# ingonyama-zk/icicle-snark

Measured on AMD Instinct MI355X. Metric: groth16_prove_constraints_per_s, higher is better.
Workload: dtype u256 mod p (MSM: 9x29-bit limbs in u32, Montgomery R=2^261, lazy reduction; NTT: 9x29-bit limbs, lazy; QAP/vec ops: 8xu32 limbs, Montgomery R=2^256)

## Files before the change

icicle-snark_amd/binding.py:

```python
from __future__ import annotations

import ctypes as C
import os

import numpy as np

_HERE = os.path.dirname(os.path.abspath(__file__))
LIB_PATH = os.path.join(_HERE, "lib", "libicicle_snark_hip.so")
os.environ.setdefault("GPU_MAX_HW_QUEUES", "12")

SUCCESS = 0
ERRORS = ["SUCCESS", "INVALID_DEVICE", "OUT_OF_MEMORY", "INVALID_POINTER", "ALLOCATION_FAILED", "DEALLOCATION_FAILED",
          "COPY_FAILED", "SYNCHRONIZATION_FAILED", "STREAM_CREATION_FAILED", "STREAM_DESTRUCTION_FAILED",
          "API_NOT_IMPLEMENTED", "INVALID_ARGUMENT", "BACKEND_LOAD_FAILED", "LICENSE_CHECK_ERROR", "UNKNOWN_ERROR"]


class IcicleError(RuntimeError):
    def __init__(self, code, what=""):
        self.code = code
        name = ERRORS[code] if 0 <= code < len(ERRORS) else str(code)
        super().__init__(f"eIcicleError::{name} {what}".strip())


class Device(C.Structure):
# ... 45 lines not shown
icicle_copy_to_host_async icicle_copy_to_device icicle_copy_to_device_async icicle_create_stream icicle_destroy_stream
icicle_stream_synchronize icicle_device_synchronize icicle_get_device_properties
create_config_extension destroy_config_extension config_extension_set_int config_extension_set_bool
config_extension_get_int config_extension_get_bool clone_config_extension
bn254_generate_scalars bn254_add bn254_sub bn254_mul bn254_inv bn254_pow bn254_from_u32
bn254_eq bn254_ecadd bn254_ecsub bn254_mul_scalar bn254_to_affine bn254_from_affine bn254_generator bn254_is_on_curve
bn254_base_field_from_u32 bn254_g2_eq bn254_g2_ecadd bn254_g2_ecsub bn254_g2_mul_scalar bn254_g2_to_affine
bn254_g2_from_affine bn254_g2_generator bn254_g2_is_on_curve bn254_g2_base_field_from_u32
bn254_vector_add bn254_vector_sub bn254_vector_mul bn254_scalar_convert_montgomery
bn254_affine_convert_montgomery bn254_g2_affine_convert_montgomery
bn254_ntt bn254_ntt_init_domain bn254_ntt_release_domain bn254_get_root_of_unity bn254_get_root_of_unity_from_domain
bn254_msm bn254_g2_msm bn254_pairing
bn254_vector_div bn254_vector_accumulate bn254_vector_sum bn254_vector_product bn254_scalar_add_vec bn254_scalar_sub_vec
bn254_scalar_mul_vec bn254_projective_convert_montgomery bn254_g2_projective_convert_montgomery
bn254_msm_precompute_bases bn254_g2_msm_precompute_bases
bn254_pairing_target_field_add bn254_pairing_target_field_sub bn254_pairing_target_field_mul bn254_pairing_target_field_inv
bn254_pairing_target_field_pow bn254_pairing_target_field_from_u32 bn254_pairing_target_field_generate_scalars
icicle_snark_last_error icicle_snark_g1_generator_mul icicle_snark_g2_generator_mul icicle_snark_last_msm_timings
icicle_snark_msm_profile icicle_snark_microbench icicle_snark_pmc_probes icicle_snark_access_probes
icicle_snark_pairing_batch icicle_snark_pairing_product icicle_snark_msm_segmented
""".split()

_lib = None


def lib():
    global _lib
    if _lib is None:
        if not os.path.exists(LIB_PATH):
            raise ImportError(f"{LIB_PATH} is missing: run `make` (hipcc --offload-arch=gfx950); "
                              "this package has no CPU fallback")
        _lib = C.CDLL(LIB_PATH)
        _lib.icicle_snark_last_error.restype = C.c_char_p
        _lib.groth16_last_error.restype = _lib.groth16_verify_last_error.restype = C.c_char_p
        _lib.groth16_cache_manager_new.restype = C.c_void_p
        _lib.groth16_zkey_export_vk.restype = C.c_int64
        _lib.groth16_verify_combined_coefficients.restype = _lib.groth16_vkset_free.restype = None
        for n in ("bn254_eq", "bn254_g2_eq", "bn254_is_on_curve", "bn254_g2_is_on_curve"):
            getattr(_lib, n).restype = C.c_bool
    return _lib


def check(rc, what=""):
    if rc != SUCCESS:
        msg = lib().icicle_snark_last_error()
        raise IcicleError(rc, f"{what}: {msg.decode() if msg else ''}")


def set_device(dev_type: str = "HIP", dev_id: int = 0):
    if dev_type != "CPU":
        check(lib().icicle_load_backend_from_env_or_default(), "load_backend")
    d = Device(dev_type.encode(), dev_id)
    check(lib().icicle_set_device(C.byref(d)), f"set_device({dev_type},{dev_id})")


def ptr_of(a):
    if a is None:
        return None
    if isinstance(a, np.ndarray):
        assert a.flags["C_CONTIGUOUS"]
        return a.ctypes.data_as(C.c_void_p)
    if isinstance(a, DeviceVec):
        return C.c_void_p(a.ptr)
    if isinstance(a, int):
        return C.c_void_p(a)
    raise TypeError(type(a))


def _on_dev(a):
    return isinstance(a, (DeviceVec, int))


class IcicleStream:

    def __init__(self, handle=None):
        if handle is None:
            h = C.c_void_p()
            check(lib().icicle_create_stream(C.byref(h)), "create_stream")
            self.handle, self._own = h.value, True
        else:
            self.handle, self._own = handle, False

    def synchronize(self):
        check(lib().icicle_stream_synchronize(C.c_void_p(self.handle)), "stream_synchronize")

    def destroy(self):
        if self._own and self.handle is not None:
            check(lib().icicle_destroy_stream(C.c_void_p(self.handle)), "destroy_stream")
            self.handle = None


class DeviceVec:

    def __init__(self, nbytes: int, stream: IcicleStream | None = None, _ptr=None, _parent=None):
        self.nbytes = nbytes
        self._parent = _parent
        if _ptr is not None:
            self.ptr = _ptr
            return
        p = C.c_void_p()
        if stream is None:
            check(lib().icicle_malloc(C.byref(p), C.c_size_t(max(nbytes, 1))), "malloc")
        else:
            check(lib().icicle_malloc_async(C.byref(p), C.c_size_t(max(nbytes, 1)), C.c_void_p(stream.handle)), "malloc_async")
        self.ptr = p.value

# ... 1402 lines not shown
```

icicle-snark_amd/csrc/common.h:

```cpp
#pragma once
#include <atomic>
#include <chrono>
#include <condition_variable>
#include <hip/hip_runtime.h>
#include <mutex>
#include <stdint.h>
#include <stdio.h>
#include <stdlib.h>
#include <string>
#include <vector>

#include "../../include/icicle_snark_hip.h"

namespace isnark {

void set_last_error(const char* fmt, ...);

inline const char* env_str(const char* name) { return getenv(name); }
inline bool env_set(const char* name) { return getenv(name) != nullptr; }
inline int env_int(const char* name, int dflt)
{
  const char* v = getenv(name);
  return v ? atoi(v) : dflt;
}
inline long long env_i64(const char* name, long long dflt)
{
  const char* v = getenv(name);
  return v ? atoll(v) : dflt;
}

inline double ms_since(std::chrono::steady_clock::time_point t0)
{
  return std::chrono::duration<double, std::milli>(std::chrono::steady_clock::now() - t0).count();
}

#define ISNARK_API extern "C" __attribute__((visibility("default")))

#define HIP_TRY(call, code)                                                                                   \
  do {                                                                                                        \
    hipError_t e__ = (call);                                                                                  \
    if (e__ != hipSuccess) {                                                                                  \
      ::isnark::set_last_error("%s failed: %s (%s:%d)", #call, hipGetErrorString(e__), __FILE__, __LINE__);   \
      return (code);                                                                                          \
    }                                                                                                         \
  } while (0)

#define ICICLE_TRY(call)                                                                                      \
  do {                                                                                                        \
    eIcicleError e__ = (call);                                                                                \
    if (e__ != ICICLE_SUCCESS) return e__;                                                                    \
  } while (0)

eIcicleError require_device();
bool is_tracked_device_ptr(const void* p);
void prewarm_device(int dev, int n_streams);
bool probe_stream_pipes(hipStream_t* st, int n, int* cls);
void stream_pipes_measure(hipStream_t* st, int n);
bool stream_pipe_classes(hipStream_t* st, int n, int* cls, bool allow_measure = true);
void stream_pipes_forget(hipStream_t st);
void prewarm_modules(int dev);
void module_warm_csr(hipStream_t s);
void module_warm_qap(hipStream_t s);
void module_warm_sort(hipStream_t s);
void module_warm_g1(hipStream_t s);
void module_warm_g2(hipStream_t s);
void module_warm_g2acc(hipStream_t s);
void module_warm_ntt(hipStream_t s);
void module_warm_vec(hipStream_t s);
int default_device_or_none();
void release_cached_device_memory();

struct CopyJob {
  void* dst;
  const void* src;
  size_t n;
};
constexpr int STAGED_LANES = 8;
constexpr size_t STAGED_CHUNK_BYTES = 2u << 20;
struct StagedProgress {
  size_t head_bytes = 0;
  hipEvent_t ev[STAGED_LANES] = {};
  std::atomic<int> lanes_total{-1};
  std::atomic<int> lanes_reported{0};
  std::atomic<bool> done{false};
  std::mutex m;
  std::condition_variable cv;
  void notify()
  {
    std::lock_guard<std::mutex> lk(m);
    cv.notify_all();
  }
  void wait_head()
  {
    std::unique_lock<std::mutex> lk(m);
    cv.wait(lk, [this] {
      const int tot = lanes_total.load(std::memory_order_acquire);
      return (tot >= 0 && lanes_reported.load(std::memory_order_acquire) >= tot) || done.load(std::memory_order_acquire);
    });
  }
};
hipError_t staged_copy(int device_id, const CopyJob* jobs, size_t njobs, bool to_device, const hipStream_t* lanes = nullptr, int n_lanes = 0, bool own_temp_streams = false,
                       StagedProgress* progress = nullptr);
void staged_copy_file_hint(const void* base, size_t len, int fd);
void staged_copy_file_hint_get(const void** base, size_t* len, int* fd);
bool is_pinned_host(const void* host_ptr, int device_id = -1);
constexpr size_t STAGED_MIN_BYTES = 4u << 20;

void note_device_write(const void* p, size_t bytes);

class Staged
{
// ... 139 lines not shown
```

icicle-snark_amd/csrc/microbench.hip:

```cpp
#include <map>
#include <string.h>
#include <mutex>

#include "common.h"

using namespace isnark;

namespace {
__global__ __launch_bounds__(256) void mad_rate_kernel(uint64_t* out, const uint32_t* in, int iters)
{
  const uint32_t a = in[threadIdx.x & 7], b = in[(threadIdx.x + 1) & 7];
  uint64_t c0 = a, c1 = b, c2 = a + 1, c3 = b + 1, c4 = 5, c5 = 6, c6 = 7, c7 = 8;
  for (int it = 0; it < iters; it++) {
#pragma unroll
    for (int u = 0; u < 8; u++) {
      c0 += (uint64_t)a * b; c1 += (uint64_t)a * b; c2 += (uint64_t)a * b; c3 += (uint64_t)a * b;
      c4 += (uint64_t)a * b; c5 += (uint64_t)a * b; c6 += (uint64_t)a * b; c7 += (uint64_t)a * b;
      asm volatile("" : "+v"(c0), "+v"(c1), "+v"(c2), "+v"(c3), "+v"(c4), "+v"(c5), "+v"(c6), "+v"(c7));
    }
  }
  out[blockIdx.x * blockDim.x + threadIdx.x] = c0 ^ c1 ^ c2 ^ c3 ^ c4 ^ c5 ^ c6 ^ c7;
}
__device__ __forceinline__ uint32_t probe_hash(uint32_t x)
{
// ... 107 lines not shown
  if (le != ICICLE_SUCCESS) return le;
  return se == hipSuccess ? ICICLE_SUCCESS : ICICLE_SYNCHRONIZATION_FAILED;
}

ISNARK_API eIcicleError icicle_snark_microbench(double out[2])
{
  if (!out) return ICICLE_INVALID_POINTER;
  ICICLE_TRY(require_device());
  hipEvent_t e0, e1;
  HIP_TRY(hipEventCreate(&e0), ICICLE_UNKNOWN_ERROR);
  HIP_TRY(hipEventCreate(&e1), ICICLE_UNKNOWN_ERROR);
  const size_t bytes = (size_t)1 << 30;
  void *a = nullptr, *b = nullptr;
  HIP_TRY(hipMalloc(&a, bytes), ICICLE_ALLOCATION_FAILED);
  HIP_TRY(hipMalloc(&b, bytes), ICICLE_ALLOCATION_FAILED);
  HIP_TRY(hipMemsetAsync(a, 1, bytes, nullptr), ICICLE_UNKNOWN_ERROR);
  HIP_TRY(hipMemcpyAsync(b, a, bytes, hipMemcpyDeviceToDevice, nullptr), ICICLE_COPY_FAILED);
  HIP_TRY(hipEventRecord(e0, nullptr), ICICLE_UNKNOWN_ERROR);
  for (int i = 0; i < 4; i++) HIP_TRY(hipMemcpyAsync(b, a, bytes, hipMemcpyDeviceToDevice, nullptr), ICICLE_COPY_FAILED);
  HIP_TRY(hipEventRecord(e1, nullptr), ICICLE_UNKNOWN_ERROR);
  HIP_TRY(hipEventSynchronize(e1), ICICLE_SYNCHRONIZATION_FAILED);
  float ms = 0;
  (void)hipEventElapsedTime(&ms, e0, e1);
  out[0] = 4.0 * 2.0 * (double)bytes / (ms * 1e-3) / 1e9;
  const int blocks = 4096, iters = 500;
  hipLaunchKernelGGL(mad_rate_kernel, dim3(blocks), dim3(256), 0, nullptr, (uint64_t*)b, (const uint32_t*)a, iters);
  HIP_TRY(hipEventRecord(e0, nullptr), ICICLE_UNKNOWN_ERROR);
  hipLaunchKernelGGL(mad_rate_kernel, dim3(blocks), dim3(256), 0, nullptr, (uint64_t*)b, (const uint32_t*)a, iters);
  HIP_TRY(hipEventRecord(e1, nullptr), ICICLE_UNKNOWN_ERROR);
  HIP_TRY(hipEventSynchronize(e1), ICICLE_SYNCHRONIZATION_FAILED);
  (void)hipEventElapsedTime(&ms, e0, e1);
  out[1] = (double)blocks * 256 * iters * 64.0 / (ms * 1e-3) / 1e12;
  (void)hipFree(a);
  (void)hipFree(b);
  (void)hipEventDestroy(e0);
  (void)hipEventDestroy(e1);
  return ICICLE_SUCCESS;
}

namespace {
__global__ __launch_bounds__(256) void pipe_probe_big_kernel(unsigned long long* out, int iters)
{
  unsigned long long x = threadIdx.x + blockIdx.x;
  for (int i = 0; i < iters; i++) x = x * 6364136223846793005ull + 1442695040888963407ull;
  if (x == 42) out[0] = x;
}
__global__ void pipe_probe_tiny_kernel(unsigned long long* out)
{
  if (threadIdx.x == 999) out[1] = 1;
}
}

namespace isnark {
bool probe_stream_pipes(hipStream_t* st, int n, int* cls)
{
  for (int i = 0; i < n; i++) cls[i] = -1;
  if (n < 2 || n > 16) return false;
  unsigned long long* d = nullptr;
  if (hipMalloc((void**)&d, 64) != hipSuccess) {
    (void)hipGetLastError();
    return false;
  }
  hipEvent_t ref = nullptr, big_end = nullptr, stop[16] = {};
  bool ok = hipEventCreate(&ref) == hipSuccess && hipEventCreate(&big_end) == hipSuccess;
  for (int i = 0; i < n && ok; i++) ok = hipEventCreate(&stop[i]) == hipSuccess;
  for (int i = 0; i < n && ok; i++) {
    hipLaunchKernelGGL(pipe_probe_tiny_kernel, dim3(1), dim3(64), 0, st[i], d);
    ok = hipStreamSynchronize(st[i]) == hipSuccess;
  }
  if (ok) {
    hipLaunchKernelGGL(pipe_probe_big_kernel, dim3(64), dim3(256), 0, st[0], d, 8);
    ok = hipStreamSynchronize(st[0]) == hipSuccess;
  }
  int next_class = 0;
  for (int x = 0; x < n && ok; x++) {
    if (cls[x] >= 0) continue;
    if (next_class >= 4) {
      ok = false;
      break;
    }
    if (next_class == 3) {
      for (int j = x; j < n; j++)
        if (cls[j] < 0) cls[j] = 3;
      break;
    }
    cls[x] = next_class;
    ok = hipEventRecord(ref, st[x]) == hipSuccess;
    hipLaunchKernelGGL(pipe_probe_big_kernel, dim3(40000), dim3(256), 0, st[x], d, 3000);
    ok = ok && hipEventRecord(big_end, st[x]) == hipSuccess;
    for (int j = 0; j < n && ok; j++) {
      if (j == x) continue;
      hipLaunchKernelGGL(pipe_probe_tiny_kernel, dim3(1), dim3(64), 0, st[j], d);
      ok = hipEventRecord(stop[j], st[j]) == hipSuccess;
    }
    for (int j = 0; j < n && ok; j++) ok = hipStreamSynchronize(st[j]) == hipSuccess;
    float big_ms = 0;
    ok = ok && hipEventElapsedTime(&big_ms, ref, big_end) == hipSuccess;
    for (int j = 0; j < n && ok; j++) {
      if (j == x) continue;
      float ms = 0;
      ok = hipEventElapsedTime(&ms, ref, stop[j]) == hipSuccess;
      const bool mate = ms > 0.35f && ms > 0.1f * big_ms;
      if (mate) {
        if (cls[j] >= 0 && cls[j] != next_class) ok = false;
        cls[j] = next_class;
      }
    }
    next_class++;
  }
  (void)hipGetLastError();
  if (ref) (void)hipEventDestroy(ref);
  if (big_end) (void)hipEventDestroy(big_end);
  for (int i = 0; i < n; i++)
    if (stop[i]) (void)hipEventDestroy(stop[i]);
  (void)hipFree(d);
  if (!ok)
    for (int i = 0; i < n; i++) cls[i] = -1;
  return ok;
}

namespace {
std::mutex g_pipe_mu;
std::map<hipStream_t, std::pair<int, int>> g_pipe_cls;
int g_pipe_epoch = 0;
}
void stream_pipes_measure(hipStream_t* st, int n)
{
  int cls[16], prev[16];
  if (n > 16) n = 16;
  bool have_prev = false, agreed = false;
  for (int attempt = 0; attempt < 4 && !agreed; attempt++) {
    if (!probe_stream_pipes(st, n, cls)) {
      have_prev = false;
      continue;
    }
    agreed = have_prev && memcmp(cls, prev, sizeof(int) * n) == 0;
    memcpy(prev, cls, sizeof(int) * n);
    have_prev = true;
  }
  if (!agreed) return;
  std::lock_guard<std::mutex> lk(g_pipe_mu);
  const int ep = ++g_pipe_epoch;
  for (int i = 0; i < n; i++) g_pipe_cls[st[i]] = {ep, cls[i]};
}
bool stream_pipe_classes(hipStream_t* st, int n, int* cls, bool allow_measure)
{
  for (int attempt = 0; attempt < (allow_measure ? 2 : 1); attempt++) {
    {
      std::lock_guard<std::mutex> lk(g_pipe_mu);
      int ep = -1;
      bool all = true;
      for (int i = 0; i < n && all; i++) {
        const auto it = g_pipe_cls.find(st[i]);
        if (it == g_pipe_cls.end() || (ep >= 0 && it->second.first != ep)) all = false;
        else {
          ep = it->second.first;
          cls[i] = it->second.second;
        }
      }
      if (all) return true;
    }
    if (attempt == 0) stream_pipes_measure(st, n);
  }
  for (int i = 0; i < n; i++) cls[i] = -1;
  return false;
}
void stream_pipes_forget(hipStream_t st)
{
  std::lock_guard<std::mutex> lk(g_pipe_mu);
  g_pipe_cls.erase(st);
}
}
```

icicle-snark_amd/csrc/prover/cache.cpp:

```cpp
#include <algorithm>
#include <utility>

#include "prover_internal.h"

using namespace bn254;
using namespace isnark;
using namespace isnark::prover;

namespace isnark {
namespace prover {

ZKeyCache::~ZKeyCache()
  {
    int prev = -1;
    if (hipGetDevice(&prev) != hipSuccess) prev = -1;
    struct Restore { int d; ~Restore() { if (d >= 0) (void)hipSetDevice(d); } } restore{prev};
    (void)hipSetDevice(device_id);
    tb.cancel.store(true);
    if (tb.th.joinable()) tb.th.join();
    for (void* t : tb.fresh)
      if (t) (void)hipFree(t);
    for (hipStream_t st : streams())
      if (st) (void)hipStreamSynchronize(st);
    for (void* p : {(void*)d_rowptr, (void*)d_cols, (void*)d_vals, A.d_points, B1.d_points, B2.d_points, C.d_points, H.d_points, (void*)d_witness, (void*)d_vec, (void*)d_fold, (void*)d_skeys, (void*)d_dist_y, (void*)d_dist_recv1, (void*)d_dist_send2, (void*)d_tw1, (void*)d_partials, (void*)d_wtnz})
      if (p) (void)hipFree(p);
    if (h_partials) (void)hipHostFree(h_partials);
    for (hipStream_t st : streams())
      if (st) (void)icicle_destroy_stream(st);
    for (hipEvent_t e : {ev_witness, ev_sort, ev_sort_h, ev_own_slice, ev_head_in, ev_head_done, ev_t_head_start, ev_t_head_end, ev_t_witness})
      if (e) (void)hipEventDestroy(e);
    for (auto e : ev)
      if (e) (void)hipEventDestroy(e);
    for (auto e : ev_done)
      if (e) (void)hipEventDestroy(e);
    for (auto e : ev_lfork)
      if (e) (void)hipEventDestroy(e);
    for (auto e : ev_ljoin)
      if (e) (void)hipEventDestroy(e);
    for (auto& p : prof) msm_profile_own_destroy(&p);
  }

namespace {
G1::P g1_from_mont_affine(const uint8_t* p)
{
  G1::A a;
  memcpy(&a, p, 64);
  if (G1::aff_is_zero(a)) return {Fq::zero(), Fq::one_std(), Fq::zero()};
  return {Fq::from_mont(a.x), Fq::from_mont(a.y), Fq::one_std()};
}
G2::P g2_from_mont_affine(const uint8_t* p)
{
  G2::A a;
  memcpy(&a, p, 128);
  fe2 one = {Fq::one_std(), Fq::zero()};
  if (G2::aff_is_zero(a)) return {Fq2Ops::zero(), one, Fq2Ops::zero()};
  return {Fq2Ops::from_mont(a.x), Fq2Ops::from_mont(a.y), one};
}

struct BaseArray {
  Shard ZKeyCache::*shard;
  int section;
  bool g2;
  bool h;
  size_t elem() const { return g2 ? 128 : 64; }
  Shard& of(ZKeyCache* z) const { return z->*shard; }
  const MsmGeom& geom(const MsmGeom& gw, const MsmGeom& gh) const { return h ? gh : gw; }
};
const BaseArray BASES[5] = {{&ZKeyCache::A, 5, false, false}, {&ZKeyCache::B1, 6, false, false}, {&ZKeyCache::B2, 7, true, false}, {&ZKeyCache::C, 8, false, false}, {&ZKeyCache::H, 9, false, true}};

uint64_t witness_row_bytes(const ZKeyCache* z) { return ((uint64_t)z->A.len() + z->B1.len() + z->C.len()) * 64 + (uint64_t)z->B2.len() * 128; }

eIcicleError points_to_internal(bool g2, const Shard& sh, int from_form, hipStream_t s)
{
  return g2 ? msm_g2_points_to_internal(sh.d_points, sh.len(), from_form, s) : msm_g1_points_to_internal(sh.d_points, sh.len(), from_form, s);
}
eIcicleError build_table(bool g2, const Shard& sh, int from_form, const MsmGeom& g, hipStream_t s, void** table)
{
  return g2 ? msm_g2_build_table(sh.d_points, sh.len(), from_form, g, s, table) : msm_g1_build_table(sh.d_points, sh.len(), from_form, g, s, table);
}
eIcicleError build_table_sliced(bool g2, const Shard& sh, int from_form, const MsmGeom& g, hipStream_t s, void** table, const std::atomic<bool>* cancel)
{
  return g2 ? msm_g2_build_table_sliced(sh.d_points, sh.len(), from_form, g, s, table, cancel) : msm_g1_build_table_sliced(sh.d_points, sh.len(), from_form, g, s, table, cancel);
}
}

int staged_upload(int device_id, const std::vector<UploadJob>& jobs, const hipStream_t* lanes_in, int n_lanes, StagedProgress* progress)
{
  const hipError_t e = staged_copy(device_id, jobs.data(), jobs.size(), true, lanes_in, n_lanes, lanes_in == nullptr, progress);
  if (e != hipSuccess) return fail((int)ICICLE_COPY_FAILED, "host to device upload: %s", hipGetErrorString(e));
  return 0;
}

MsmGeom witness_table_geometry(uint32_t len)
{
  MsmGeom g = msm_geometry(len, 0, 1);
  if (!g.tab) return g;
  int c = g.c;
  while (c > 17 && (((uint64_t)len * (uint64_t)(254 / c + 1)) >> (c - 1)) < 28) c--;
  if (c != g.c) {
    const MsmGeom h = msm_geometry(len, 0, c);
    if (h.tab && h.c == c) return h;
  }
  return g;
}

namespace {
void assign_stream_roles(ZKeyCache* z, bool allow_measure)
{
  static const bool off = env_int("ICICLE_SNARK_PIPE_ROLES", 1) == 0;
  if (off) return;
  std::array<hipStream_t, 6> phys = z->streams();
  int cls[6];
  if (!stream_pipe_classes(phys.data(), 6, cls, allow_measure)) return;
  auto cost = [&](const int* perm) {
    auto same = [&](int a, int b) { return cls[perm[a]] == cls[perm[b]] ? 1 : 0; };
    int c = 1000 * (same(0, 2) + same(0, 3) + same(2, 3)) + 200 * (same(2, 1) + same(2, 4) + same(2, 5) + same(3, 1) + same(3, 4) + same(3, 5)) + 100 * (1 - same(0, 4)) +
            100 * (1 - same(1, 5));
    for (int r = 0; r < 6; r++) c += perm[r] != r ? 1 : 0;
    return c;
  };
  int perm[6] = {0, 1, 2, 3, 4, 5}, best[6] = {0, 1, 2, 3, 4, 5};
  int best_cost = cost(perm);
  while (std::next_permutation(perm, perm + 6)) {
    const int c = cost(perm);
    if (c < best_cost) {
      best_cost = c;
      memcpy(best, perm, sizeof best);
    }
  }
  int r = 0;
  for (hipStream_t* role : {&z->s_qap, &z->s_g1, &z->s_g2, &z->s_g3, &z->s_g4, &z->s_g5}) *role = phys[best[r++]];
  if (env_set("ICICLE_SNARK_TRACE_COLD") || env_set("ICICLE_SNARK_VERBOSE"))
    fprintf(stderr, "[icicle-snark-hip] stream pipes %d %d %d %d %d %d -> roles (qap A B2 Hsort B1 C) take streams %d %d %d %d %d %d (cost %d)\n", cls[0], cls[1], cls[2], cls[3], cls[4], cls[5], best[0],
            best[1], best[2], best[3], best[4], best[5], best_cost);
}
}

namespace {
void table_build_thread(ZKeyCache* z)
{
  TableBuild& tb = z->tb;
  while (tb.hold.load(std::memory_order_acquire) && !tb.cancel.load()) std::this_thread::sleep_for(std::chrono::milliseconds(1));
  const int grace_ms = env_int("ICICLE_SNARK_TABLE_GRACE_MS", TABLE_BUILD_GRACE_MS);
  for (int waited = 0; !tb.witness_only && waited < grace_ms && !tb.go.load(std::memory_order_acquire) && !tb.cancel.load(); waited++) std::this_thread::sleep_for(std::chrono::milliseconds(1));
  const auto t0 = std::chrono::steady_clock::now();
  static const bool trace_tb = env_set("ICICLE_SNARK_TRACE_TABLES");
  bool ok = hipSetDevice(z->device_id) == hipSuccess;
  if (trace_tb) fprintf(stderr, "[tables] thread: device set at %.1f ms\n", ms_since(t0));
  const MsmGeom gw_dense = tb.gw;
  bool narrowed = false;
  if (ok && !tb.witness_only && tb.go.load(std::memory_order_acquire) && z->witness_entries) {
    int lg = 0;
    while (((uint64_t)1 << lg) * 32 < z->witness_entries) lg++;
    int c_t = lg + 1 < 13 ? 13 : lg + 1;
    if (c_t < tb.gw.c) {
      const MsmGeom g = msm_geometry(z->A.len(), 0, c_t);
      if (g.tab && g.c == c_t && g.W > tb.gw.W) {
        const uint64_t per_row = witness_row_bytes(z);
        const uint64_t extra = (uint64_t)(g.W - tb.gw.W) * per_row;
        size_t free_b = 0, total_b = 0;
        const bool mem_ok = hipMemGetInfo(&free_b, &total_b) == hipSuccess && (uint64_t)g.W * per_row + (uint64_t)tb.gh.W * z->H.len() * 64 + (1ull << 30) <= free_b;
        (void)hipGetLastError();
        if (mem_ok && extra <= tb.narrow_room.load(std::memory_order_acquire)) {
          tb.gw = g;
          tb.extra_bytes.store(extra, std::memory_order_release);
          narrowed = true;
        }
      } else if (g.tab && g.c == c_t)
        tb.gw = g;
    }
  }
  hipStream_t s = nullptr;
  if (ok) {
    int least = 0, greatest = 0;
    if (hipDeviceGetStreamPriorityRange(&least, &greatest) != hipSuccess) least = 0;
    if (hipStreamCreateWithPriority(&s, hipStreamNonBlocking, least) != hipSuccess) {
      (void)hipGetLastError();
      ok = false;
    }
  }
  if (trace_tb) fprintf(stderr, "[tables] thread: stream created at %.1f ms\n", ms_since(t0));
  const int order[5] = {4, 0, 1, 3, 2};
  for (int attempt = 0; attempt < 2; attempt++) {
    for (int k : order) {
      const BaseArray& b = BASES[k];
      if (b.h && tb.witness_only) continue;
      if (b.h && tb.fresh[k]) continue;
// ... 565 lines not shown
```

icicle-snark_amd/csrc/runtime.cpp:

```cpp
#include <atomic>
#include <map>
#include <thread>
#include <execinfo.h>
#include <mutex>
#include <signal.h>
#include <vector>
#include <stdarg.h>
#include <string.h>
#include <unistd.h>
#include <chrono>

#include "common.h"
#include "msm_plan.h"
#include "workers.h"

static void isnark_segv(int sig)
{
  void* frames[64];
  const int n = backtrace(frames, 64);
  backtrace_symbols_fd(frames, n, 2);
  signal(sig, SIG_DFL);
  raise(sig);
}
__attribute__((constructor)) static void isnark_runtime_env()
// ... 893 lines not shown
  return ICICLE_SUCCESS;
}
ISNARK_API eIcicleError icicle_copy_to_device_async(void* dst, const void* src, size_t size, icicleStreamHandle stream)
{
  ICICLE_TRY(require_device());
  note_device_write(dst, size);
  bool done;
  ICICLE_TRY(big_pageable_copy(dst, src, size, true, (hipStream_t)stream, &done));
  if (!done) HIP_TRY(hipMemcpyAsync(dst, src, size, hipMemcpyHostToDevice, (hipStream_t)stream), ICICLE_COPY_FAILED);
  return ICICLE_SUCCESS;
}

constexpr size_t STREAM_POOL_MAX = 10;
ISNARK_API eIcicleError icicle_create_stream(icicleStreamHandle* stream)
{
  if (!stream) return ICICLE_INVALID_POINTER;
  ICICLE_TRY(require_device());
  {
    std::lock_guard<std::mutex> lk(g_sp_mu);
    std::vector<hipStream_t>& v = g_stream_pool[t_device];
    if (!v.empty()) {
      *stream = v.back();
      v.pop_back();
      return ICICLE_SUCCESS;
    }
  }
  hipStream_t s;
  HIP_TRY(hipStreamCreateWithFlags(&s, hipStreamNonBlocking), ICICLE_STREAM_CREATION_FAILED);
  *stream = s;
  return ICICLE_SUCCESS;
}
ISNARK_API eIcicleError icicle_destroy_stream(icicleStreamHandle stream)
{
  if (!stream) return ICICLE_SUCCESS;
  HIP_TRY(hipStreamSynchronize((hipStream_t)stream), ICICLE_STREAM_DESTRUCTION_FAILED);
  {
    int d = 0;
    hipDevice_t sd = 0;
    if (hipStreamGetDevice((hipStream_t)stream, &sd) == hipSuccess) d = (int)sd;
    else (void)hipGetDevice(&d);
    std::lock_guard<std::mutex> lk(g_sp_mu);
    std::vector<hipStream_t>& v = g_stream_pool[d];
    if (v.size() < STREAM_POOL_MAX) {
      v.push_back((hipStream_t)stream);
      return ICICLE_SUCCESS;
    }
  }
  ws_release_stream((hipStream_t)stream);
  stream_pipes_forget((hipStream_t)stream);
  HIP_TRY(hipStreamDestroy((hipStream_t)stream), ICICLE_STREAM_DESTRUCTION_FAILED);
  return ICICLE_SUCCESS;
}
namespace isnark {
void prewarm_device(int dev, int n_streams)
{
  if (dev < 0 || dev >= STAGED_DEVICES || hipSetDevice(dev) != hipSuccess) {
    (void)hipGetLastError();
    return;
  }
  {
    StagedPool& P = g_staged[dev];
    std::lock_guard<std::mutex> lk(P.mu);
    if (staged_pool_init(P) != hipSuccess) (void)hipGetLastError();
  }
  size_t have = 0;
  {
    std::lock_guard<std::mutex> lk(g_sp_mu);
    have = g_stream_pool[dev].size();
  }
  const size_t warm_bytes = g_staged[dev].pinned ? STAGED_CHUNK : 4096;
  void* d = nullptr;
  if (hipMalloc(&d, warm_bytes) != hipSuccess) {
    (void)hipGetLastError();
    return;
  }
  std::vector<hipStream_t> fresh;
  for (size_t k = have; k < (size_t)n_streams && k < STREAM_POOL_MAX; k++) {
    hipStream_t st;
    if (hipStreamCreateWithFlags(&st, hipStreamNonBlocking) != hipSuccess) break;
    (void)hipMemcpyAsync(d, g_staged[dev].pinned ? (void*)g_staged[dev].pinned : d, warm_bytes, g_staged[dev].pinned ? hipMemcpyHostToDevice : hipMemcpyDeviceToDevice, st);
    fresh.push_back(st);
  }
  for (hipStream_t st : fresh) (void)hipStreamSynchronize(st);
  (void)hipFree(d);
  (void)hipGetLastError();
  static const bool pipe_roles = env_int("ICICLE_SNARK_PIPE_ROLES", 1) != 0;
  if (pipe_roles && fresh.size() >= 2) stream_pipes_measure(fresh.data(), (int)fresh.size());
  std::lock_guard<std::mutex> lk(g_sp_mu);
  std::vector<hipStream_t>& v = g_stream_pool[dev];
  for (hipStream_t st : fresh) {
    if (v.size() < STREAM_POOL_MAX) v.push_back(st);
    else (void)hipStreamDestroy(st);
  }
}
void prewarm_modules(int dev)
{
  if (dev < 0 || hipSetDevice(dev) != hipSuccess) {
    (void)hipGetLastError();
    return;
  }
  hipStream_t s = nullptr;
  if (hipStreamCreateWithFlags(&s, hipStreamNonBlocking) != hipSuccess) {
    (void)hipGetLastError();
    return;
  }
  module_warm_csr(s);
  module_warm_qap(s);
  module_warm_sort(s);
  module_warm_g1(s);
  module_warm_g2(s);
  module_warm_g2acc(s);
  module_warm_ntt(s);
  module_warm_vec(s);
  (void)hipStreamSynchronize(s);
  (void)hipStreamDestroy(s);
  (void)hipGetLastError();
}
int default_device_or_none() { return active_device(); }
}

ISNARK_API eIcicleError icicle_stream_synchronize(icicleStreamHandle stream)
{
  ICICLE_TRY(require_device());
  HIP_TRY(hipStreamSynchronize((hipStream_t)stream), ICICLE_SYNCHRONIZATION_FAILED);
  return ICICLE_SUCCESS;
}
ISNARK_API eIcicleError icicle_device_synchronize(void)
{
  ICICLE_TRY(require_device());
  HIP_TRY(hipDeviceSynchronize(), ICICLE_SYNCHRONIZATION_FAILED);
  return ICICLE_SUCCESS;
}

ISNARK_API eIcicleError icicle_get_device_properties(IcicleDeviceProperties* p)
{
  if (!p) return ICICLE_INVALID_POINTER;
  ICICLE_TRY(require_device());
  p->using_host_memory = false;
  p->num_memory_regions = 0;
  p->supports_pinned_memory = true;
  return ICICLE_SUCCESS;
}

struct ConfigExtension {
  std::map<std::string, int> ints;
  std::map<std::string, bool> bools;
};
ISNARK_API ConfigExtension* create_config_extension(void) { return new ConfigExtension(); }
ISNARK_API void destroy_config_extension(ConfigExtension* ext) { delete ext; }
ISNARK_API void config_extension_set_int(ConfigExtension* ext, const char* key, int value)
{
  if (ext && key) ext->ints[key] = value;
}
ISNARK_API void config_extension_set_bool(ConfigExtension* ext, const char* key, bool value)
{
  if (ext && key) ext->bools[key] = value;
}
ISNARK_API int config_extension_get_int(const ConfigExtension* ext, const char* key)
{
  if (!ext || !key) { set_last_error("ConfigExtension is null"); return 0; }
  auto it = ext->ints.find(key);
  if (it == ext->ints.end()) { set_last_error("ConfigExtension: no int key '%s'", key); return 0; }
  return it->second;
}
ISNARK_API bool config_extension_get_bool(const ConfigExtension* ext, const char* key)
{
  if (!ext || !key) { set_last_error("ConfigExtension is null"); return false; }
  auto it = ext->bools.find(key);
  if (it == ext->bools.end()) { set_last_error("ConfigExtension: no bool key '%s'", key); return false; }
  return it->second;
}
ISNARK_API ConfigExtension* clone_config_extension(const ConfigExtension* ext)
{
// ... 23 lines not shown
```

include/groth16_prover.h:

```cpp
#ifndef GROTH16_PROVER_H
#define GROTH16_PROVER_H

#include <stddef.h>
#include <stdint.h>

#ifdef __cplusplus
extern "C" {
#endif

typedef struct Groth16CacheManager Groth16CacheManager;

Groth16CacheManager* groth16_cache_manager_new(void);
void groth16_cache_manager_free(Groth16CacheManager* cm);
void groth16_cache_manager_prewarm(Groth16CacheManager* cm, int device_id);

int groth16_prove(const char* witness_path, const char* zkey_path, const char* proof_path, const char* public_path,
                  const char* device, Groth16CacheManager* cm);


int groth16_cache_load(Groth16CacheManager* cm, const char* key, const void* zkey, size_t zkey_len, int device_id,
                       int shard_rank, int shard_count);
int groth16_cache_load_file(Groth16CacheManager* cm, const char* key, const char* zkey_path, int device_id,
                            int shard_rank, int shard_count);
int groth16_cache_tables_ready(Groth16CacheManager* cm, const char* key, int wait);
int groth16_cache_load_devices(Groth16CacheManager* cm, const char* key, const void* zkey, size_t zkey_len, const int* device_ids,
                               int n_devices);
int groth16_parse_device(const char* device, int* ids, int cap);
void groth16_cache_set_budget(Groth16CacheManager* cm, uint64_t bytes_per_device);
int groth16_cache_contains(const Groth16CacheManager* cm, const char* key);
void groth16_cache_evict(Groth16CacheManager* cm, const char* key);

#define GROTH16_COMMITMENTS_BYTES 576
typedef struct {
  double h2d_ms;
  double qap_ms;
  double msm_ms;
  double total_ms;
} Groth16Timings;
int groth16_commitments(Groth16CacheManager* cm, const char* key, const void* wtns, size_t wtns_len,
                        uint8_t out_points[GROTH16_COMMITMENTS_BYTES], Groth16Timings* timings );

int groth16_upload_witness_slice(Groth16CacheManager* cm, const char* key, const void* wtns, size_t wtns_len, void** d_witness, uint64_t* slice_bytes);
int groth16_witness_ready(Groth16CacheManager* cm, const char* key);

int groth16_dist_supported(Groth16CacheManager* cm, const char* key);
int groth16_dist_stage1(Groth16CacheManager* cm, const char* key, const void* wtns, size_t wtns_len, void** d_send,
                        void** d_recv, uint32_t* rows, uint64_t* row_bytes, uint64_t* chunk_bytes);
int groth16_dist_stage2(Groth16CacheManager* cm, const char* key, void** d_send, void** d_recv);
int groth16_dist_exchange_done(Groth16CacheManager* cm, const char* key);

int groth16_sum_commitments(const uint8_t* blocks, int count, uint8_t out_points[GROTH16_COMMITMENTS_BYTES]);

int groth16_assemble_proof(Groth16CacheManager* cm, const char* key, const void* wtns, size_t wtns_len,
                           const uint8_t points[GROTH16_COMMITMENTS_BYTES], const uint8_t* r, const uint8_t* s,
                           char* proof_json, size_t proof_cap, char* public_json, size_t public_cap);

int groth16_prove_mem(Groth16CacheManager* cm, const char* key, const void* wtns, size_t wtns_len, const uint8_t* r,
                      const uint8_t* s, char* proof_json, size_t proof_cap, char* public_json, size_t public_cap,
                      Groth16Timings* timings);

int groth16_prove_resident(Groth16CacheManager* cm, const char* key, const void* wtns, size_t wtns_len, int wtns_resident,
                           const uint8_t* r, const uint8_t* s, char* proof_json, size_t proof_cap, char* public_json,
                           size_t public_cap, Groth16Timings* timings);

typedef struct {
  uint32_t n_vars, n_public, domain_size, n_coef;
  uint64_t device_bytes;
  uint32_t b_bases;
  uint32_t shards;
} Groth16CircuitInfo;
int groth16_cache_info(const Groth16CacheManager* cm, const char* key, Groth16CircuitInfo* info);
int groth16_cache_info_sized(const Groth16CacheManager* cm, const char* key, void* info, size_t info_size);

int groth16_group_describe(const Groth16CacheManager* cm, const char* key, char* out, size_t cap);

int groth16_last_timings(Groth16CacheManager* cm, const char* key, Groth16Timings* timings);

const char* groth16_last_error(void);

int groth16_verify(const char* proof_path, const char* public_path, const char* vk_path);
int groth16_verify_json(const char* proof_json, const char* public_json, const char* vk_json);
// ... 381 lines not shown
```

Baseline: 100.5 million.

## Probe hardware queue sharing among streams and swap duplicates for distinct-queue streams

Extends the stream pipe probe so it also detects which streams share a hardware queue, by checking whether a tiny kernel finishes after a big kernel on another stream. Before measuring, the six prover role streams are checked for shared queues, and a stream on a duplicate queue is replaced with a pooled stream on a queue not yet used. The aim is to stop role streams from serialising behind each other on the same hardware queue. It also adds a stream_plan header (a queue-aware role planner, not yet wired in beyond the pipe deal) and a Python probe binding. The extra probing makes cold setup more expensive, and the probe may misclassify streams.

Result: no change. 100.3 million (median of 2 runs) (-0.3%).

```diff
diff --git a/icicle-snark_amd/binding.py b/icicle-snark_amd/binding.py
--- a/icicle-snark_amd/binding.py
+++ b/icicle-snark_amd/binding.py
@@ -121,6 +121,12 @@
         check(lib().icicle_load_backend_from_env_or_default(), "load_backend")
     d = Device(dev_type.encode(), dev_id)
     check(lib().icicle_set_device(C.byref(d)), f"set_device({dev_type},{dev_id})")
+
+
+def probe_stream_pool(cap: int = 16):
+    q, p = (C.c_int * 16)(), (C.c_int * 16)()
+    n = lib().icicle_snark_probe_stream_pool(q, p, min(cap, 16))
+    return list(q)[:n], list(p)[:n]
 
 
 def ptr_of(a):
diff --git a/icicle-snark_amd/csrc/common.h b/icicle-snark_amd/csrc/common.h
--- a/icicle-snark_amd/csrc/common.h
+++ b/icicle-snark_amd/csrc/common.h
@@ -54,9 +54,11 @@
 eIcicleError require_device();
 bool is_tracked_device_ptr(const void* p);
 void prewarm_device(int dev, int n_streams);
-bool probe_stream_pipes(hipStream_t* st, int n, int* cls);
+bool probe_stream_pipes(hipStream_t* st, int n, int* cls, int* qcls);
 void stream_pipes_measure(hipStream_t* st, int n);
-bool stream_pipe_classes(hipStream_t* st, int n, int* cls, bool allow_measure = true);
+bool stream_pipe_classes(hipStream_t* st, int n, int* cls, int* qcls, bool allow_measure = true);
+bool stream_class_lookup(hipStream_t st, int* epoch, int* pipe, int* queue);
+hipStream_t stream_pool_take_if(int dev, bool (*want)(hipStream_t, void*), void* arg);
 void stream_pipes_forget(hipStream_t st);
 void prewarm_modules(int dev);
 void module_warm_csr(hipStream_t s);
diff --git a/icicle-snark_amd/csrc/microbench.hip b/icicle-snark_amd/csrc/microbench.hip
--- a/icicle-snark_amd/csrc/microbench.hip
+++ b/icicle-snark_amd/csrc/microbench.hip
@@ -183,9 +183,9 @@
 }
 
 namespace isnark {
-bool probe_stream_pipes(hipStream_t* st, int n, int* cls)
-{
-  for (int i = 0; i < n; i++) cls[i] = -1;
+bool probe_stream_pipes(hipStream_t* st, int n, int* cls, int* qcls)
+{
+  for (int i = 0; i < n; i++) cls[i] = qcls[i] = -1;
   if (n < 2 || n > 16) return false;
   unsigned long long* d = nullptr;
   if (hipMalloc((void**)&d, 64) != hipSuccess) {
@@ -203,7 +203,30 @@
     hipLaunchKernelGGL(pipe_probe_big_kernel, dim3(64), dim3(256), 0, st[0], d, 8);
     ok = hipStreamSynchronize(st[0]) == hipSuccess;
   }
-  int next_class = 0;
+  bool late[16], behind[16];
+  auto round = [&](int x, unsigned others) {
+    ok = hipEventRecord(ref, st[x]) == hipSuccess;
+    hipLaunchKernelGGL(pipe_probe_big_kernel, dim3(40000), dim3(256), 0, st[x], d, 3000);
+    ok = ok && hipEventRecord(big_end, st[x]) == hipSuccess;
+    for (int j = 0; j < n && ok; j++) {
+      if (!((others >> j) & 1)) continue;
+      hipLaunchKernelGGL(pipe_probe_tiny_kernel, dim3(1), dim3(64), 0, st[j], d);
+      ok = hipEventRecord(stop[j], st[j]) == hipSuccess;
+    }
+    for (int j = 0; j < n && ok; j++) ok = hipStreamSynchronize(st[j]) == hipSuccess;
+    float big_ms = 0;
+    ok = ok && hipEventElapsedTime(&big_ms, ref, big_end) == hipSuccess;
+    for (int j = 0; j < n && ok; j++) {
+      late[j] = behind[j] = false;
+      if (!((others >> j) & 1)) continue;
+      float ms = 0, after = 0;
+      ok = hipEventElapsedTime(&ms, ref, stop[j]) == hipSuccess && hipEventElapsedTime(&after, big_end, stop[j]) == hipSuccess;
+      behind[j] = ok && after >= 0;
+      late[j] = behind[j] || (ms > 0.35f && ms > 0.1f * big_ms);
+    }
+  };
+  const unsigned all = (1u << n) - 1;
+  int next_class = 0, next_queue = 0;
   for (int x = 0; x < n && ok; x++) {
     if (cls[x] >= 0) continue;
     if (next_class >= 4) {
@@ -216,28 +239,35 @@
       break;
     }
     cls[x] = next_class;
-    ok = hipEventRecord(ref, st[x]) == hipSuccess;
-    hipLaunchKernelGGL(pipe_probe_big_kernel, dim3(40000), dim3(256), 0, st[x], d, 3000);
-    ok = ok && hipEventRecord(big_end, st[x]) == hipSuccess;
+    qcls[x] = next_queue++;
+    round(x, all & ~(1u << x));
     for (int j = 0; j < n && ok; j++) {
-      if (j == x) continue;
-      hipLaunchKernelGGL(pipe_probe_tiny_kernel, dim3(1), dim3(64), 0, st[j], d);
-      ok = hipEventRecord(stop[j], st[j]) == hipSuccess;
-    }
-    for (int j = 0; j < n && ok; j++) ok = hipStreamSynchronize(st[j]) == hipSuccess;
-    float big_ms = 0;
-    ok = ok && hipEventElapsedTime(&big_ms, ref, big_end) == hipSuccess;
-    for (int j = 0; j < n && ok; j++) {
-      if (j == x) continue;
-      float ms = 0;
-      ok = hipEventElapsedTime(&ms, ref, stop[j]) == hipSuccess;
-      const bool mate = ms > 0.35f && ms > 0.1f * big_ms;
-      if (mate) {
-        if (cls[j] >= 0 && cls[j] != next_class) ok = false;
-        cls[j] = next_class;
-      }
+      if (j == x || !late[j]) continue;
+      if (cls[j] >= 0 && cls[j] != next_class) ok = false;
+      cls[j] = next_class;
+      if (behind[j]) qcls[j] = qcls[x];
     }
     next_class++;
+  }
+  for (int x = 0; x < n && ok; x++) {
+    if (qcls[x] >= 0) continue;
+    qcls[x] = next_queue++;
+    unsigned open = 0;
+    for (int j = x + 1; j < n; j++)
+      if (cls[j] == cls[x] && qcls[j] < 0) open |= 1u << j;
+    if (!open) continue;
+    round(x, open);
+    for (int j = 0; j < n && ok; j++)
+      if (((open >> j) & 1) && behind[j]) qcls[j] = qcls[x];
+  }
+  for (int i = 0; i < n && ok; i++) ok = cls[i] >= 0 && qcls[i] >= 0;
+  if (ok) {
+    int relabel[16], next = 0;
+    for (int i = 0; i < 16; i++) relabel[i] = -1;
+    for (int i = 0; i < n; i++) {
+      if (relabel[qcls[i]] < 0) relabel[qcls[i]] = next++;
+      qcls[i] = relabel[qcls[i]];
+    }
   }
   (void)hipGetLastError();
   if (ref) (void)hipEventDestroy(ref);
@@ -246,35 +276,38 @@
     if (stop[i]) (void)hipEventDestroy(stop[i]);
   (void)hipFree(d);
   if (!ok)
-    for (int i = 0; i < n; i++) cls[i] = -1;
+    for (int i = 0; i < n; i++) cls[i] = qcls[i] = -1;
   return ok;
 }
 
 namespace {
 std::mutex g_pipe_mu;
-std::map<hipStream_t, std::pair<int, int>> g_pipe_cls;
+struct StreamClass {
+  int epoch, pipe, queue;
+};
+std::map<hipStream_t, StreamClass> g_pipe_cls;
 int g_pipe_epoch = 0;
 }
 void stream_pipes_measure(hipStream_t* st, int n)
 {
-  int cls[16], prev[16];
+  int cls[32], prev[32];
   if (n > 16) n = 16;
   bool have_prev = false, agreed = false;
   for (int attempt = 0; attempt < 4 && !agreed; attempt++) {
-    if (!probe_stream_pipes(st, n, cls)) {
+    if (!probe_stream_pipes(st, n, cls, cls + 16)) {
       have_prev = false;
       continue;
     }
-    agreed = have_prev && memcmp(cls, prev, sizeof(int) * n) == 0;
-    memcpy(prev, cls, sizeof(int) * n);
+    agreed = have_prev && memcmp(cls, prev, sizeof(int) * n) == 0 && memcmp(cls + 16, prev + 16, sizeof(int) * n) == 0;
+    memcpy(prev, cls, sizeof cls);
     have_prev = true;
   }
   if (!agreed) return;
   std::lock_guard<std::mutex> lk(g_pipe_mu);
   const int ep = ++g_pipe_epoch;
-  for (int i = 0; i < n; i++) g_pipe_cls[st[i]] = {ep, cls[i]};
-}
-bool stream_pipe_classes(hipStream_t* st, int n, int* cls, bool allow_measure)
+  for (int i = 0; i < n; i++) g_pipe_cls[st[i]] = {ep, cls[i], cls[16 + i]};
+}
+bool stream_pipe_classes(hipStream_t* st, int n, int* cls, int* qcls, bool allow_measure)
 {
   for (int attempt = 0; attempt < (allow_measure ? 2 : 1); attempt++) {
     {
@@ -283,18 +316,27 @@
       bool all = true;
       for (int i = 0; i < n && all; i++) {
         const auto it = g_pipe_cls.find(st[i]);
-        if (it == g_pipe_cls.end() || (ep >= 0 && it->second.first != ep)) all = false;
+        if (it == g_pipe_cls.end() || (ep >= 0 && it->second.epoch != ep)) all = false;
         else {
-          ep = it->second.first;
-          cls[i] = it->second.second;
+          ep = it->second.epoch;
+          cls[i] = it->second.pipe;
+          qcls[i] = it->second.queue;
         }
       }
       if (all) return true;
     }
     if (attempt == 0) stream_pipes_measure(st, n);
   }
-  for (int i = 0; i < n; i++) cls[i] = -1;
+  for (int i = 0; i < n; i++) cls[i] = qcls[i] = -1;
   return false;
+}
+bool stream_class_lookup(hipStream_t st, int* epoch, int* pipe, int* queue)
+{
+  std::lock_guard<std::mutex> lk(g_pipe_mu);
+  const auto it = g_pipe_cls.find(st);
+  if (it == g_pipe_cls.end()) return false;
+  *epoch = it->second.epoch, *pipe = it->second.pipe, *queue = it->second.queue;
+  return true;
 }
 void stream_pipes_forget(hipStream_t st)
 {
diff --git a/icicle-snark_amd/csrc/prover/cache.cpp b/icicle-snark_amd/csrc/prover/cache.cpp
--- a/icicle-snark_amd/csrc/prover/cache.cpp
+++ b/icicle-snark_amd/csrc/prover/cache.cpp
@@ -2,6 +2,7 @@
 #include <utility>
 
 #include "prover_internal.h"
+#include "stream_plan.h"
 
 using namespace bn254;
 using namespace isnark;
@@ -105,34 +106,54 @@
 }
 
 namespace {
+struct WantQueue {
+  int epoch;
+  const int* have;
+  int n_have;
+};
+bool want_new_queue(hipStream_t s, void* arg)
+{
+  const WantQueue* w = (const WantQueue*)arg;
+  int ep, pipe, queue;
+  if (!stream_class_lookup(s, &ep, &pipe, &queue) || ep != w->epoch) return false;
+  for (int i = 0; i < w->n_have; i++)
+    if (w->have[i] == queue) return false;
+  return true;
+}
+void cover_queues(ZKeyCache* z)
+{
+  hipStream_t* member[SP_N] = {&z->s_qap, &z->s_g1, &z->s_g2, &z->s_g3, &z->s_g4, &z->s_g5};
+  for (int round = 0; round < SP_N; round++) {
+    int ep[SP_N], pipe, q[SP_N];
+    for (int i = 0; i < SP_N; i++)
+      if (!stream_class_lookup(*member[i], &ep[i], &pipe, &q[i]) || ep[i] != ep[0]) return;
+    int dup = -1;
+    for (int i = 1; i < SP_N && dup < 0; i++)
+      for (int j = 0; j < i; j++)
+        if (q[j] == q[i]) dup = i;
+    if (dup < 0) return;
+    WantQueue w{ep[0], q, SP_N};
+    hipStream_t fresh = stream_pool_take_if(z->device_id, want_new_queue, &w);
+    if (!fresh) return;
+    (void)icicle_destroy_stream((icicleStreamHandle)*member[dup]);
+    *member[dup] = fresh;
+  }
+}
 void assign_stream_roles(ZKeyCache* z, bool allow_measure)
 {
   static const bool off = env_int("ICICLE_SNARK_PIPE_ROLES", 1) == 0;
   if (off) return;
+  if (allow_measure) cover_queues(z);
   std::array<hipStream_t, 6> phys = z->streams();
-  int cls[6];
-  if (!stream_pipe_classes(phys.data(), 6, cls, allow_measure)) return;
-  auto cost = [&](const int* perm) {
-    auto same = [&](int a, int b) { return cls[perm[a]] == cls[perm[b]] ? 1 : 0; };
-    int c = 1000 * (same(0, 2) + same(0, 3) + same(2, 3)) + 200 * (same(2, 1) + same(2, 4) + same(2, 5) + same(3, 1) + same(3, 4) + same(3, 5)) + 100 * (1 - same(0, 4)) +
-            100 * (1 - same(1, 5));
-    for (int r = 0; r < 6; r++) c += perm[r] != r ? 1 : 0;
-    return c;
-  };
-  int perm[6] = {0, 1, 2, 3, 4, 5}, best[6] = {0, 1, 2, 3, 4, 5};
-  int best_cost = cost(perm);
-  while (std::next_permutation(perm, perm + 6)) {
-    const int c = cost(perm);
-    if (c < best_cost) {
-      best_cost = c;
-      memcpy(best, perm, sizeof best);
-    }
-  }
+  int cls[6], qcls[6];
+  if (!stream_pipe_classes(phys.data(), 6, cls, qcls, allow_measure)) return;
+  int best[6];
+  const int best_cost = stream_plan_pipe_deal(cls, best);
   int r = 0;
   for (hipStream_t* role : {&z->s_qap, &z->s_g1, &z->s_g2, &z->s_g3, &z->s_g4, &z->s_g5}) *role = phys[best[r++]];
   if (env_set("ICICLE_SNARK_TRACE_COLD") || env_set("ICICLE_SNARK_VERBOSE"))
-    fprintf(stderr, "[icicle-snark-hip] stream pipes %d %d %d %d %d %d -> roles (qap A B2 Hsort B1 C) take streams %d %d %d %d %d %d (cost %d)\n", cls[0], cls[1], cls[2], cls[3], cls[4], cls[5], best[0],
-            best[1], best[2], best[3], best[4], best[5], best_cost);
+    fprintf(stderr, "[icicle-snark-hip] stream queues %d %d %d %d %d %d pipes %d %d %d %d %d %d -> roles (qap A B2 Hsort B1 C) take streams %d %d %d %d %d %d (cost %d)\n", qcls[0], qcls[1], qcls[2], qcls[3],
+            qcls[4], qcls[5], cls[0], cls[1], cls[2], cls[3], cls[4], cls[5], best[0], best[1], best[2], best[3], best[4], best[5], best_cost);
 }
 }
 
diff --git a/icicle-snark_amd/csrc/prover/stream_plan.h b/icicle-snark_amd/csrc/prover/stream_plan.h
--- /dev/null
+++ b/icicle-snark_amd/csrc/prover/stream_plan.h
@@ -0,0 +1,195 @@
+#pragma once
+#include <stdint.h>
+#include <string.h>
+
+#include <algorithm>
+#include <initializer_list>
+
+namespace isnark {
+
+constexpr int SP_N = 6;
+
+enum SpRole {
+  SP_FRONT = 0,
+  SP_A, SP_B1, SP_B2, SP_C,
+  SP_H,
+  SP_WSORT,
+  SP_HEAD,
+  SP_HSORT,
+  SP_SIDE_A, SP_SIDE_B1, SP_SIDE_B2, SP_SIDE_C, SP_SIDE_H,
+  SP_LANE0, SP_LANE1, SP_LANE2,
+  SP_ROLES
+};
+constexpr int SP_INLINE = -1;
+constexpr int SP_SIDE_DEFAULT = 0x14;
+
+constexpr SpRole SP_CHAIN[4] = {SP_A, SP_B1, SP_B2, SP_C};
+
+struct SpShape {
+  bool early = false;
+  bool head = false;
+  bool h_chain = false;
+  bool cold = false;
+  bool shard = false;
+  int side_mask = SP_SIDE_DEFAULT;
+};
+
+enum SpStage {
+  SG_UP_HEAD0 = 0, SG_UP_HEAD1, SG_UP_HEAD2,
+  SG_HEAD,
+  SG_UP_TAIL0, SG_UP_TAIL1, SG_UP_TAIL2,
+  SG_FRONT, SG_WSORT, SG_HSORT,
+  SG_ACC0, SG_ACC1, SG_ACC2, SG_ACC3, SG_ACC4,
+  SG_SIDE0, SG_SIDE1, SG_SIDE2, SG_SIDE3, SG_SIDE4,
+  SG_RED0, SG_RED1, SG_RED2, SG_RED3, SG_RED4,
+  SG_COPY_B1,
+  SG_STAGES
+};
+constexpr int SP_MAX_WAIT = 4;
+
+struct SpStageAt {
+  int stage = -1;
+  int nwait = 0;
+  int wait[SP_MAX_WAIT] = {-1, -1, -1, -1};
+};
+
+struct StreamPlan {
+  bool identity = true;
+  int nqueues = 0;
+  int slot[SP_N];
+  int stream[SP_ROLES];
+  int n_order = 0;
+  int order[SG_STAGES];
+  int n_on[SP_N];
+  SpStageAt on[SP_N][SG_STAGES];
+};
+
+inline int stream_plan_pipe_deal(const int* pipe, int* best)
+{
+  auto cost = [&](const int* perm) {
+    auto same = [&](int a, int b) { return pipe[perm[a]] == pipe[perm[b]] ? 1 : 0; };
+    int c = 1000 * (same(0, 2) + same(0, 3) + same(2, 3)) + 200 * (same(2, 1) + same(2, 4) + same(2, 5) + same(3, 1) + same(3, 4) + same(3, 5)) + 100 * (1 - same(0, 4)) +
+            100 * (1 - same(1, 5));
+    for (int r = 0; r < SP_N; r++) c += perm[r] != r ? 1 : 0;
+    return c;
+  };
+  int perm[SP_N] = {0, 1, 2, 3, 4, 5};
+  for (int r = 0; r < SP_N; r++) best[r] = r;
+  int best_cost = cost(perm);
+  while (std::next_permutation(perm, perm + SP_N)) {
+    const int c = cost(perm);
+    if (c < best_cost) {
+      best_cost = c;
+      memcpy(best, perm, sizeof perm);
+    }
+  }
+  return best_cost;
+}
+
+namespace stream_plan_detail {
+inline void add_stage(StreamPlan& p, int stage, int stream, std::initializer_list<int> waits)
+{
+  p.order[p.n_order++] = stage;
+  SpStageAt& s = p.on[stream][p.n_on[stream]++];
+  s.stage = stage;
+  for (int w : waits)
+    if (w >= 0 && s.nwait < SP_MAX_WAIT) s.wait[s.nwait++] = w;
+}
+}
+
+inline StreamPlan stream_plan(const int* queue_cls, const int* pipe_cls, const SpShape& shape)
+{
+  SpShape sh = shape;
+  if (sh.cold) sh.head = false;
+  StreamPlan p;
+  for (int i = 0; i < SP_N; i++) p.slot[i] = i, p.n_on[i] = 0;
+  bool measured = true;
+  for (int i = 0; i < SP_N; i++) measured = measured && queue_cls[i] >= 0 && pipe_cls[i] >= 0;
+  int rep[SP_N], nq = 0;
+  if (measured) {
+    for (int i = 0; i < SP_N; i++) {
+      bool seen = false;
+      for (int j = 0; j < i; j++) seen = seen || queue_cls[j] == queue_cls[i];
+      if (!seen) rep[nq++] = i;
+    }
+  }
+  p.nqueues = nq;
+  int sF = 0, sA = 1, sB2 = 2, sHS = 3, sB1 = 4, sC = 5, sTail = 3;
+  bool folded = false;
+  if (measured && (nq >= SP_N || sh.shard)) {
+    stream_plan_pipe_deal(pipe_cls, p.slot);
+    p.identity = false;
+  } else if (measured) {
+    bool used[SP_N] = {};
+    int k = 0;
+    for (; k < nq; k++) p.slot[k] = rep[k], used[rep[k]] = true;
+    for (int i = 0; i < SP_N; i++)
+      if (!used[i]) p.slot[k++] = i;
+    folded = true;
+    p.identity = false;
+    if (nq >= 4) {
+      sF = sB1 = 0, sA = 1, sB2 = 2, sC = sTail = 3;
+      sHS = nq >= 5 ? 4 : 3;
+    } else if (nq == 3) {
+      sF = sB1 = 0, sA = sC = sHS = sTail = 1, sB2 = 2;
+    } else if (nq == 2) {
+      sF = sB1 = sB2 = 0, sA = sC = sHS = sTail = 1;
+    } else
+      sF = sB1 = sB2 = sA = sC = sHS = sTail = 0;
+  }
+  int* st = p.stream;
+  st[SP_FRONT] = p.slot[sF];
+  st[SP_A] = p.slot[sA];
+  st[SP_B1] = p.slot[sB1];
+  st[SP_B2] = p.slot[sB2];
+  st[SP_C] = p.slot[sC];
+  st[SP_HSORT] = p.slot[sHS];
+  st[SP_H] = sh.h_chain ? st[SP_B1] : st[SP_HSORT];
+  st[SP_HEAD] = st[SP_B2];
+  st[SP_WSORT] = sh.head ? p.slot[sTail] : st[SP_B2];
+  for (int k = 0; k < 5; k++) {
+    int side = SP_INLINE;
+    if (!folded && ((sh.side_mask >> k) & 1) && !(k == 4 && !sh.h_chain)) side = k >= 3 ? st[SP_HSORT] : st[SP_FRONT];
+    st[SP_SIDE_A + k] = side;
+  }
+  if (folded) {
+    st[SP_LANE0] = st[SP_FRONT];
+    st[SP_LANE1] = st[SP_A];
+    st[SP_LANE2] = st[SP_C];
+  } else if (sh.head) {
+    st[SP_LANE0] = st[SP_FRONT], st[SP_LANE1] = st[SP_HSORT], st[SP_LANE2] = st[SP_C];
+  } else
+    st[SP_LANE0] = st[SP_FRONT], st[SP_LANE1] = st[SP_B2], st[SP_LANE2] = st[SP_HSORT];
+
+  using stream_plan_detail::add_stage;
+  const bool up = !sh.cold;
+  if (up && sh.head) {
+    for (int l = 0; l < 3; l++) add_stage(p, SG_UP_HEAD0 + l, st[SP_LANE0 + l], {});
+    add_stage(p, SG_HEAD, st[SP_HEAD], {SG_UP_HEAD0, SG_UP_HEAD1, SG_UP_HEAD2});
+  }
+  if (up)
+    for (int l = 0; l < 3; l++) add_stage(p, SG_UP_TAIL0 + l, st[SP_LANE0 + l], {});
+  const int w0 = up ? SG_UP_TAIL0 : -1, w1 = up ? SG_UP_TAIL1 : -1, w2 = up ? SG_UP_TAIL2 : -1;
+  if (sh.early) add_stage(p, SG_WSORT, st[SP_WSORT], {w0, w1, w2});
+  add_stage(p, SG_FRONT, st[SP_FRONT], {w0, w1, w2});
+  if (!sh.early) add_stage(p, SG_WSORT, st[SP_WSORT], {w0, w1, w2});
+  auto msm = [&](int k) {
+    const int chain = k < 4 ? st[SP_CHAIN[k]] : st[SP_H];
+    if (k < 4) add_stage(p, SG_ACC0 + k, chain, {SG_WSORT, sh.early ? -1 : SG_FRONT, sh.head && k != 2 ? SG_HEAD : -1});
+    else add_stage(p, SG_ACC0 + k, chain, {sh.h_chain ? SG_HSORT : -1});
+    const int side = st[SP_SIDE_A + k];
+    if (side != SP_INLINE) add_stage(p, SG_SIDE0 + k, side, {SG_ACC0 + k});
+    add_stage(p, SG_RED0 + k, chain, {side != SP_INLINE ? SG_SIDE0 + k : -1});
+  };
+  if (sh.cold) add_stage(p, SG_HSORT, st[SP_HSORT], {SG_FRONT});
+  msm(2);
+  if (!sh.cold) add_stage(p, SG_HSORT, st[SP_HSORT], {SG_FRONT});
+  msm(0);
+  msm(1);
+  msm(3);
+  msm(4);
+  if (sh.h_chain) add_stage(p, SG_COPY_B1, st[SP_HSORT], {SG_RED1});
+  return p;
+}
+
+}
diff --git a/icicle-snark_amd/csrc/runtime.cpp b/icicle-snark_amd/csrc/runtime.cpp
--- a/icicle-snark_amd/csrc/runtime.cpp
+++ b/icicle-snark_amd/csrc/runtime.cpp
@@ -969,6 +969,22 @@
   return ICICLE_SUCCESS;
 }
 namespace isnark {
+hipStream_t stream_pool_take_if(int dev, bool (*want)(hipStream_t, void*), void* arg)
+{
+  std::lock_guard<std::mutex> lk(g_sp_mu);
+  auto it = g_stream_pool.find(dev);
+  if (it == g_stream_pool.end()) return nullptr;
+  std::vector<hipStream_t>& v = it->second;
+  for (size_t i = 0; i < v.size(); i++)
+    if (want(v[i], arg)) {
+      hipStream_t s = v[i];
+      v.erase(v.begin() + i);
+      return s;
+    }
+  return nullptr;
+}
+}
+namespace isnark {
 void prewarm_device(int dev, int n_streams)
 {
   if (dev < 0 || dev >= STAGED_DEVICES || hipSetDevice(dev) != hipSuccess) {
@@ -1036,6 +1052,27 @@
 int default_device_or_none() { return active_device(); }
 }
 
+extern "C" __attribute__((visibility("default"))) int icicle_snark_probe_stream_pool(int* queue_cls, int* pipe_cls, int cap)
+{
+  if (!queue_cls || !pipe_cls || require_device() != ICICLE_SUCCESS) return 0;
+  std::vector<hipStream_t> v;
+  {
+    std::lock_guard<std::mutex> lk(g_sp_mu);
+    v = g_stream_pool[t_device];
+    g_stream_pool[t_device].clear();
+  }
+  int n = (int)v.size() < cap ? (int)v.size() : cap;
+  if (n > 16) n = 16;
+  bool ok = false;
+  for (int attempt = 0; attempt < 4 && !ok && n >= 2; attempt++) ok = isnark::probe_stream_pipes(v.data(), n, pipe_cls, queue_cls);
+  {
+    std::lock_guard<std::mutex> lk(g_sp_mu);
+    std::vector<hipStream_t>& pool = g_stream_pool[t_device];
+    pool.insert(pool.begin(), v.begin(), v.end());
+  }
+  return ok ? n : 0;
+}
+
 ISNARK_API eIcicleError icicle_stream_synchronize(icicleStreamHandle stream)
 {
   ICICLE_TRY(require_device());
diff --git a/include/groth16_prover.h b/include/groth16_prover.h
--- a/include/groth16_prover.h
+++ b/include/groth16_prover.h
@@ -27,6 +27,7 @@
                                int n_devices);
 int groth16_parse_device(const char* device, int* ids, int cap);
 void groth16_cache_set_budget(Groth16CacheManager* cm, uint64_t bytes_per_device);
+int icicle_snark_probe_stream_pool(int* queue_cls, int* pipe_cls, int cap);
 int groth16_cache_contains(const Groth16CacheManager* cm, const char* key);
 void groth16_cache_evict(Groth16CacheManager* cm, const char* key);
 
```
